# intel/rho-diffusion

Measured on AMD Instinct MI355X. Metric: denoising_steps_per_sec, higher is better.
Workload: dtype bf16; 1 GPU; DDPM reverse step, UNetv2 3D 64^3 mc=64 (BASELINE configs[2]), batch 32/GPU, bf16, LinearSchedule(1000,1e-3,0.02); global_batch=32, hip_graph=True

## Files before the change

### rho_diffusion_amd/csrc/conv.hip

```cpp
#include <cstdio>
#include <cstdlib>
#include <type_traits>

#include "conv_common.h"

#define RHO_GB_WIDE 3
#ifndef RHO_GB_BM32
#define RHO_GB_BM32 1
#endif

struct ConvK {
    const char* x1;
    const char* x2;
    const float* pre_a;
    const float* pre_b;
    const char* w;
    const float* bias;
    const char* res;
    const float* res_add;
    char* y;
    char* y2;
    int c1, c2, cin;
    int cout, coutp, split;
    int D, H, W;
// ... 984 lines not shown
                float accv = 0.0f;
                for (int q = 0; q < NTHR / PPR; ++q) accv += red[(q * PPR + piece) * (2 * PE) + e2];
                const int stat = e2 / PE, ch = co0 + piece * PE + (e2 % PE);
                q.stats[(((size_t)ns * q.tps + ts) * 2 + stat) * q.split + ch] = accv;
            }
        }
        return;
    }
#pragma unroll
    for (int jx = 0; jx < (M16 ? 4 : 2); ++jx) {
        const int pp = M16 ? tile_position16(wpos * 4 + jx, lane & 15, q.TW, q.pair_lg) : tile_position(wpos * 2 + jx, lane & 31, q.TW, q.pair_lg);
        const int pw = pp & (q.TW - 1);
        const int ph = (pp >> q.lgTW) & (q.TH - 1);
        const int pd = pp >> (q.lgTW + q.lgTH);
        const int od = od0 + pd, oh = oh0 + ph, ow = ow0 + pw;
        if (od >= q.Do || oh >= q.Ho || ow >= q.Wo) continue;
        const long long L = (((long long)n * q.Do + od) * q.Ho + oh) * q.Wo + ow;
        const long long ns = L / q.S_out;
        const long long ps = L - ns * q.S_out;
        const int j = M16 ? (jx >> 1) : jx;
#pragma unroll
        for (int mi = 0; mi < MT; ++mi) {
#pragma unroll
            for (int rx = 0; rx < (M16 ? 2 : 4); ++rx) {
                const int rg = M16 ? 2 * rx + (jx & 1) : rx;
                const int co = M16 ? co0 + wco * (BM / WCO) + 16 * (2 * mi + rx) + 4 * (lane >> 4)
                                   : co0 + wco * (BM / WCO) + mi * 32 + rg * 8 + half * 4;
                const float4 bv = *reinterpret_cast<const float4*>(q.bias + co);
                float v0 = acc[mi][j][rg * 4 + 0] + bv.x;
                float v1 = acc[mi][j][rg * 4 + 1] + bv.y;
                float v2 = acc[mi][j][rg * 4 + 2] + bv.z;
                float v3 = acc[mi][j][rg * 4 + 3] + bv.w;
                if (cl_region) {
                    if (q.res_add != nullptr) {
                        const float4 e = *reinterpret_cast<const float4*>(q.res_add + ns * q.res_add_stride + co);
                        v0 += e.x; v1 += e.y; v2 += e.z; v3 += e.w;
                    }
                    const size_t eo = (size_t)L * q.split + co;
                    if constexpr (sizeof(T) == 2) {
                        if (q.res != nullptr) {
                            const uint2 r = *reinterpret_cast<const uint2*>(q.res + eo * 2);
                            v0 += __uint_as_float(r.x << 16); v1 += __uint_as_float(r.x & 0xFFFF0000u);
                            v2 += __uint_as_float(r.y << 16); v3 += __uint_as_float(r.y & 0xFFFF0000u);
                        }
                        *reinterpret_cast<uint2*>(q.y + eo * 2) = make_uint2(pack_bf16x2(v0, v1), pack_bf16x2(v2, v3));
                    } else {
                        if (q.res != nullptr) {
                            const float4 r = *reinterpret_cast<const float4*>(q.res + eo * 4);
                            v0 += r.x; v1 += r.y; v2 += r.z; v3 += r.w;
                        }
                        *reinterpret_cast<float4*>(q.y + eo * 4) = make_float4(v0, v1, v2, v3);
                    }
                } else if (q.y2_cl) {
                    const int w2 = q.cout - q.split;
                    const size_t eo = (size_t)L * w2 + (co - q.split);
                    if (co < q.cout) {
                        if constexpr (sizeof(T) == 2) {
                            if (q.res2 != nullptr) {
                                const uint2 r = *reinterpret_cast<const uint2*>(q.res2 + eo * 2);
                                v0 += __uint_as_float(r.x << 16); v1 += __uint_as_float(r.x & 0xFFFF0000u);
                                v2 += __uint_as_float(r.y << 16); v3 += __uint_as_float(r.y & 0xFFFF0000u);
                            }
                            *reinterpret_cast<uint2*>(q.y2 + eo * 2) = make_uint2(pack_bf16x2(v0, v1), pack_bf16x2(v2, v3));
                        } else {
                            if (q.res2 != nullptr) {
                                const float4 r = *reinterpret_cast<const float4*>(q.res2 + eo * 4);
                                v0 += r.x; v1 += r.y; v2 += r.z; v3 += r.w;
                            }
                            *reinterpret_cast<float4*>(q.y2 + eo * 4) = make_float4(v0, v1, v2, v3);
                        }
                    }
                } else {
                    const float vv[4] = {v0, v1, v2, v3};
#pragma unroll
                    for (int e = 0; e < 4; ++e) {
                        if (co + e < q.cout) {
                            const size_t eo = ((size_t)ns * (q.cout - q.split) + (co + e - q.split)) * q.S_out + ps;
                            if (q.y2_f32 || sizeof(T) == 4)
                                reinterpret_cast<float*>(q.y2)[eo] = vv[e];
                            else
                                reinterpret_cast<bf16_raw*>(q.y2)[eo] = f32_to_bf16(vv[e]);
                        }
                    }
                }
            }
        }
    }
}

struct SplitMap {
    int Ho, Wo, Ho_out, Wo_out, oy_mul, oy_add, ox_mul, ox_add;
};
struct SplitOut {
    int cout, coutp, split;
    const float* bias;
    const float* res_add;
    long long res_add_stride, S_out;
    const char* res;
    char* y;
    const char* res2;
    char* y2;
};
template <typename T>
__global__ __launch_bounds__(256) void k_splitk_reduce(const float* __restrict__ slab, long long slab_stride, int ksplit, long long positions,
                                                       SplitOut o, SplitMap m) {
    const int c4 = o.coutp / 4;
    const long long item = (long long)blockIdx.x * 256 + threadIdx.x;
    if (item >= positions * c4) return;
    const long long Ls = item / c4;
    int co = (int)(item - Ls * c4) * 4;
    if (co >= o.cout) return;
    const size_t so = (size_t)Ls * o.coutp + co;
    float4 a = *reinterpret_cast<const float4*>(slab + so);
    for (int s = 1; s < ksplit; ++s) {
        const float4 b = *reinterpret_cast<const float4*>(slab + (size_t)s * slab_stride + so);
        a.x += b.x; a.y += b.y; a.z += b.z; a.w += b.w;
    }
    long long L = Ls;
    if (m.oy_mul != 1 || m.ox_mul != 1) {
        const int ow = (int)(Ls % m.Wo);
        const long long r = Ls / m.Wo;
        const int oh = (int)(r % m.Ho);
        L = ((r / m.Ho) * m.Ho_out + (oh * m.oy_mul + m.oy_add)) * m.Wo_out + (ow * m.ox_mul + m.ox_add);
    }
    const float4 bv = *reinterpret_cast<const float4*>(o.bias + co);
    float v0 = a.x + bv.x, v1 = a.y + bv.y, v2 = a.z + bv.z, v3 = a.w + bv.w;
    const bool first = co < o.split;
    if (first && o.res_add != nullptr) {
        const float4 e = *reinterpret_cast<const float4*>(o.res_add + (L / o.S_out) * o.res_add_stride + co);
        v0 += e.x; v1 += e.y; v2 += e.z; v3 += e.w;
    }
    const int width = first ? o.split : o.cout - o.split;
    const char* const res = first ? o.res : o.res2;
    char* const y = first ? o.y : o.y2;
    if (!first) co -= o.split;
    const size_t eo = (size_t)L * width + co;
    if constexpr (sizeof(T) == 2) {
        if (res != nullptr) {
            const uint2 r = *reinterpret_cast<const uint2*>(res + eo * 2);
            v0 += __uint_as_float(r.x << 16); v1 += __uint_as_float(r.x & 0xFFFF0000u);
            v2 += __uint_as_float(r.y << 16); v3 += __uint_as_float(r.y & 0xFFFF0000u);
        }
        *reinterpret_cast<uint2*>(y + eo * 2) = make_uint2(pack_bf16x2(v0, v1), pack_bf16x2(v2, v3));
    } else {
        if (res != nullptr) {
            const float4 r = *reinterpret_cast<const float4*>(res + eo * 4);
            v0 += r.x; v1 += r.y; v2 += r.z; v3 += r.w;
        }
        *reinterpret_cast<float4*>(y + eo * 4) = make_float4(v0, v1, v2, v3);
    }
}

#include "conv32.h"

namespace {

using namespace rho_conv;

struct VariantOut {
    char* buf;
    int cap;
};
thread_local VariantOut* g_variant = nullptr;

template <typename T, int KD, int KH, int KW, int BM, int MAXP, int NW, bool M16 = false, bool FSK = false, bool GNA = false>
int launch_one(const ConvK& k, dim3 grid, size_t lds, hipStream_t st) {
    if (g_variant != nullptr) {
        snprintf(g_variant->buf, (size_t)g_variant->cap, "k_conv<%s,%d,%d,%d,BM=%d,MAXP=%d,NW=%d,M16=%d>%s%s", sizeof(T) == 2 ? "bf16" : "f32",
                 KD, KH, KW, BM, MAXP, NW, (int)M16, FSK ? "+skip" : "", GNA ? "+gn_apply" : "");
        return 0;
    }
    auto fn = k_conv<T, KD, KH, KW, BM, MAXP, NW, M16, FSK, GNA>;
    if (lds > 64 * 1024) {
        hipError_t e = hipFuncSetAttribute(reinterpret_cast<const void*>(fn), hipFuncAttributeMaxDynamicSharedMemorySize, (int)lds);
        if (e != hipSuccess) return (int)e;
    }
    hipLaunchKernelGGL(fn, grid, dim3(NW * 64), lds, st, k);
    hipError_t e = hipGetLastError();
    return e == hipSuccess ? 0 : (int)e;
}

template <typename T, int KD, int KH, int KW>
int launch_bm(const ConvK& k, int BM, int np, dim3 grid, size_t lds, bool m16, hipStream_t st) {
    constexpr bool PHASE = (KH == 2 || KW == 2 || (KD == 3 && KH == 1 && KW == 1));
    if constexpr (PHASE) { if (np > 640) return RHO_E_SHAPE; }
    if constexpr (sizeof(T) == 2 && KD * KH * KW > 1 && (KD * KH * KW) % 3 == 0) {
        if (m16 && np <= 640) {
            if constexpr (KD == 3 && KH == 3 && KW == 3) {
                if (k.sk_w != nullptr) {
                    if (BM == 128) return launch_one<T, KD, KH, KW, 128, 5, 8, true, true>(k, grid, lds, st);
                    if (BM == 64) return launch_one<T, KD, KH, KW, 64, 10, 4, true, true>(k, grid, lds, st);
                }
            }
            if (BM == 128) return launch_one<T, KD, KH, KW, 128, 5, 8, true>(k, grid, lds, st);
            if (BM == 64) return launch_one<T, KD, KH, KW, 64, 10, 4, true>(k, grid, lds, st);
        }
    }
    if (k.sk_w != nullptr) return RHO_E_ARG;
    if (k.gna_g != nullptr) {
        if constexpr (KD * KH * KW == 1) {
            if (np > 640) return RHO_E_SHAPE;
            if (BM == 128) return launch_one<T, 1, 1, 1, 128, 5, 8, false, false, true>(k, grid, lds, st);
            if (BM == 64) return launch_one<T, 1, 1, 1, 64, 10, 4, false, false, true>(k, grid, lds, st);
            return launch_one<T, 1, 1, 1, 32, 10, 4, false, false, true>(k, grid, lds, st);
        }
        return RHO_E_ARG;
    }
    if (BM == 128) {
        if (np <= 640) return launch_one<T, KD, KH, KW, 128, 5, 8>(k, grid, lds, st);
        if constexpr (!PHASE) return launch_one<T, KD, KH, KW, 128, 14, 8>(k, grid, lds, st);
    }
#define RHO_CASE(bm)                                                                   \
    if (BM == bm) {                                                                    \
        if (np <= 640) return launch_one<T, KD, KH, KW, bm, 10, 4>(k, grid, lds, st);  \
        if constexpr (!PHASE) return launch_one<T, KD, KH, KW, bm, 28, 4>(k, grid, lds, st); \
    }
    RHO_CASE(32)
    RHO_CASE(64)
#undef RHO_CASE
    return RHO_E_ARG;
}

template <typename T>
int launch_taps(const rho_conv_desc& d, const ConvK& k, int BM, int np, dim3 grid, size_t lds, bool m16, hipStream_t st) {
    if (d.kd == 3 && d.kh == 3 && d.kw == 3) return launch_bm<T, 3, 3, 3>(k, BM, np, grid, lds, m16, st);
    if (d.kd == 1 && d.kh == 3 && d.kw == 3) return launch_bm<T, 1, 3, 3>(k, BM, np, grid, lds, m16, st);
    if (d.kd == 1 && d.kh == 1 && d.kw == 3) return launch_bm<T, 1, 1, 3>(k, BM, np, grid, lds, m16, st);
    if (d.kd == 1 && d.kh == 1 && d.kw == 1) return launch_bm<T, 1, 1, 1>(k, BM, np, grid, lds, m16, st);
    if (d.kd == 3 && d.kh == 2 && d.kw == 2) return launch_bm<T, 3, 2, 2>(k, BM, np, grid, lds, m16, st);
    if (d.kd == 1 && d.kh == 2 && d.kw == 2) return launch_bm<T, 1, 2, 2>(k, BM, np, grid, lds, m16, st);
    if (d.kd == 1 && d.kh == 1 && d.kw == 2) return launch_bm<T, 1, 1, 2>(k, BM, np, grid, lds, m16, st);
    if (d.kd == 3 && d.kh == 1 && d.kw == 1) return launch_bm<T, 3, 1, 1>(k, BM, np, grid, lds, m16, st);
    if (d.kd == 3 && d.kh == 1 && d.kw == 2) return launch_bm<T, 3, 1, 2>(k, BM, np, grid, lds, m16, st);
    if (d.kd == 3 && d.kh == 2 && d.kw == 1) return launch_bm<T, 3, 2, 1>(k, BM, np, grid, lds, m16, st);
    return RHO_E_ARG;
}

}

static bool m16_env_on() {
    static const bool on = !(getenv("RHO_CONV_M16") && atoi(getenv("RHO_CONV_M16")) == 0);
    return on;
}

static int conv_impl(const rho_conv_desc* dp, void* stream, int64_t* stats_tiles, int64_t* ws_want = nullptr) {
    if (!dp) return RHO_E_ARG;
    const rho_conv_desc& d = *dp;
    if (!d.x1 || !d.w || !d.bias) return RHO_E_ARG;
    if (d.dtype != RHO_F32 && d.dtype != RHO_BF16) return RHO_E_ARG;
    const int CK = d.dtype == RHO_BF16 ? 32 : 16;
    const int c2 = d.x2 ? d.c2 : 0;
    const int cin = d.c1 + c2;
    if (d.c1 <= 0 || d.c1 % CK || c2 % CK) return RHO_E_ALIGN;
    if (d.cout <= 0 || d.coutp < d.cout || d.coutp % 32 || d.split < 0 || d.split > d.cout || d.split % 32) return RHO_E_ARG;
    if (d.split > 0 && !d.y) return RHO_E_ARG;
    if (d.split < d.cout && !d.y2) return RHO_E_ARG;
    if (d.split < d.cout && d.split > 0 && d.coutp != d.cout && !d.y2_cl) return RHO_E_ARG;
    if (d.y2_cl && ((d.cout - d.split) % 4 != 0)) return RHO_E_ALIGN;
    if ((d.zs_h || d.zs_w) && (d.up_h || d.up_w || d.sh != 1 || d.sw != 1 || d.out_h <= 0 || d.out_w <= 0)) return RHO_E_ARG;
    if (d.split == d.cout && d.coutp != d.cout) return RHO_E_ARG;
    if ((d.sh != 1 && d.sh != 2) || (d.sw != 1 && d.sw != 2)) return RHO_E_ARG;
    if ((d.up_h && d.sh != 1) || (d.up_w && d.sw != 1)) return RHO_E_ARG;
    if ((d.up_h && d.kh != 3) || (d.up_w && d.kw != 3)) return RHO_E_ARG;
    if (d.n <= 0 || d.d <= 0 || d.h <= 0 || d.w_ <= 0) return RHO_E_ARG;
    if (d.ph_h < 0 || d.ph_h > 2 || d.ph_w < 0 || d.ph_w > 2) return RHO_E_ARG;
    if ((d.ph_h && ((d.kh != 2 && d.kh != 1) || d.sh != 1 || d.up_h || d.zs_h)) || (d.ph_w && ((d.kw != 2 && d.kw != 1) || d.sw != 1 || d.up_w || d.zs_w)))
        return RHO_E_ARG;
    if ((!d.ph_h && !d.phd_h && d.kh == 2) || (!d.ph_w && !d.phd_w && d.kw == 2)) return RHO_E_ARG;
    if ((d.ph_h || d.ph_w) && (d.split != d.cout || d.kd == 2)) return RHO_E_ARG;
    if (d.phd_h < 0 || d.phd_h > 2 || d.phd_w < 0 || d.phd_w > 2) return RHO_E_ARG;
    if ((d.phd_h && ((d.kh != 2 && d.kh != 1) || d.sh != 1 || d.up_h || d.zs_h || d.ph_h)) ||
        (d.phd_w && ((d.kw != 2 && d.kw != 1) || d.sw != 1 || d.up_w || d.zs_w || d.ph_w)))
        return RHO_E_ARG;
    if ((d.ph_h || d.phd_h || d.ph_w || d.phd_w) && d.kd * d.kh * d.kw == 1) return RHO_E_ARG;
    if ((d.phd_h || d.phd_w) && (d.kd == 2 || d.pre_a)) return RHO_E_ARG;

    if (conv32_applies(d)) {
        if (stats_tiles) { *stats_tiles = conv32_wps(d); return 0; }
        if (ws_want) { *ws_want = 0; return 0; }
        if (g_variant != nullptr) { snprintf(g_variant->buf, (size_t)g_variant->cap, "k_conv32<bf16>"); return 0; }
        if (d.stats && d.split != d.cout) return RHO_E_ARG;
        return launch_conv32(d, as_stream(stream));
    }

    const int hv = d.zs_h ? d.out_h : d.h, wv = d.zs_w ? d.out_w : d.w_;
    const int ho = (d.ph_h || d.phd_h) ? d.h : d.up_h ? d.h * 2 : (hv + 2 * (d.kh / 2) - d.kh) / d.sh + 1;
    const int wo = (d.ph_w || d.phd_w) ? d.w_ : d.up_w ? d.w_ * 2 : (wv + 2 * (d.kw / 2) - d.kw) / d.sw + 1;
    const int ho_out = d.ph_h ? 2 * ho : ho, wo_out = d.ph_w ? 2 * wo : wo;
    const int n_phase = (d.ph_h ? 2 : 1) * (d.ph_w ? 2 : 1);
    const int phase_idx = (d.ph_h ? d.ph_h - 1 : 0) * (d.ph_w ? 2 : 1) + (d.ph_w ? d.ph_w - 1 : 0);
    const int dout = d.d;

    ConvK k{};
    int gridz = d.n;
    k.pad_h = d.kh == 1 ? 0 : d.ph_h ? 2 - d.ph_h : d.phd_h ? d.phd_h - 1 : d.kh / 2;
    k.pad_w = d.kw == 1 ? 0 : d.ph_w ? 2 - d.ph_w : d.phd_w ? d.phd_w - 1 : d.kw / 2;
    k.iy_mul = d.phd_h ? 2 : 1; k.iy_add = d.phd_h ? d.phd_h - 1 : 0;
    k.ix_mul = d.phd_w ? 2 : 1; k.ix_add = d.phd_w ? d.phd_w - 1 : 0;
    k.oy_mul = d.ph_h ? 2 : 1; k.oy_add = d.ph_h ? d.ph_h - 1 : 0;
    k.ox_mul = d.ph_w ? 2 : 1; k.ox_add = d.ph_w ? d.ph_w - 1 : 0;
    if (d.kd == 1 && d.kh == 1 && d.kw == 1) {
        if (d.sh != 1 || d.sw != 1 || d.up_h || d.up_w) return RHO_E_ARG;
        k.D = 1; k.H = 1; k.W = d.n * d.d * d.h * d.w_;
        k.Do = 1; k.Ho = 1; k.Wo = k.W;
        gridz = 1;
    } else if (d.kd == 1) {
        k.D = d.n * d.d; k.H = hv; k.W = wv;
        k.Do = k.D; k.Ho = ho; k.Wo = wo;
        gridz = 1;
    } else {
        k.D = d.d; k.H = hv; k.W = wv;
        k.Do = dout; k.Ho = ho; k.Wo = wo;
    }
    k.Hs = k.H; k.Ws = k.W;
    if (d.zs_h) k.Hs = d.h;
    if (d.zs_w) k.Ws = d.w_;
    if (d.phd_h) k.Hs = 2 * d.h;
    if (d.phd_w) k.Ws = 2 * d.w_;
    k.zs_h = d.zs_h; k.zs_w = d.zs_w;
    k.y2_cl = d.y2_cl; k.res2 = (const char*)d.res2;
    if ((long long)d.n * d.d * d.h * d.w_ * (d.phd_h ? 2 : 1) * (d.phd_w ? 2 : 1) >= (1LL << 31) || (long long)d.n * dout * ho_out * wo_out >= (1LL << 31)) return RHO_E_SHAPE;
    k.S_in = (long long)d.d * d.h * d.w_ * (d.phd_h ? 2 : 1) * (d.phd_w ? 2 : 1);
    k.S_out = (long long)dout * ho_out * wo_out;
    k.Ho_out = (d.kd == 1 && d.kh == 1 && d.kw == 1) ? 1 : ho_out;
    k.Wo_out = (d.kd == 1 && d.kh == 1 && d.kw == 1) ? k.Wo : wo_out;

    int BM = 32;
    if (d.coutp % 128 == 0 && (d.split % 128 == 0)) BM = 128;
    else if (d.coutp % 64 == 0 && (d.split % 64 == 0)) BM = 64;

    const size_t lds_cap = 160 * 1024;
    const int taps = d.kd * d.kh * d.kw;
    {
        static const int bm64_chunks = getenv("RHO_BM64_MAX_CHUNKS") ? atoi(getenv("RHO_BM64_MAX_CHUNKS")) : 0;
        if (BM == 128 && bm64_chunks > 0 && d.kd == 3 && taps > 1 && cin / CK <= bm64_chunks) BM = 64;
    }
    const bool m16 = d.dtype == RHO_BF16 && taps > 1 && taps % 3 == 0 && d.sh == 1 && d.sw == 1 && !d.up_h && !d.up_w;
    const int WSLOTS = (taps % 3 == 0) ? ((((BM == 128 && m16) || (RHO_GB_BM32 && BM == 32)) && RHO_GB_WIDE == 3 && taps % 9 == 0) ? 9 : 3) : 2;
    int np_cap = (int)((lds_cap - (size_t)WSLOTS * BM * PITCH) / PITCH);
    if (np_cap > 28 * 64) np_cap = 28 * 64;
    TileChoice t = choose_tile(d, k.D, k.Do, k.Ho, k.Wo, 640);
    if (!t.ok) t = choose_tile(d, k.D, k.Do, k.Ho, k.Wo, np_cap);
    if (!t.ok) return RHO_E_SHAPE;

    k.x1 = (const char*)d.x1; k.x2 = (const char*)d.x2; k.pre_a = d.pre_a; k.pre_b = d.pre_b;
    k.w = (const char*)d.w; k.bias = d.bias; k.res = (const char*)d.res; k.res_add = d.res_add;
    k.y = (char*)d.y; k.y2 = (char*)d.y2;
    k.c1 = d.c1; k.c2 = c2; k.cin = cin;
    k.cout = d.cout; k.coutp = d.coutp; k.split = d.split;
    k.res_add_stride = d.res_add_stride > 0 ? d.res_add_stride : d.split;
    k.sh = d.sh; k.sw = d.sw; k.up_h = d.up_h; k.up_w = d.up_w; k.pre_silu = d.pre_silu; k.y2_f32 = d.y2_f32;
    k.TD = t.TD; k.TH = t.TH; k.TW = t.TW; k.ID = t.ID; k.IH = t.IH; k.IW = t.IW; k.NP = t.NP;
    k.tiles_h = cdiv(k.Ho, t.TH); k.tiles_w = cdiv(k.Wo, t.TW);
    k.lgTW = 0; k.lgTH = 0;
    while ((1 << k.lgTW) < t.TW) ++k.lgTW;
    while ((1 << k.lgTH) < t.TH) ++k.lgTH;
    if ((1 << k.lgTW) != t.TW || (1 << k.lgTH) != t.TH) return RHO_E_SHAPE;
    k.inv_ihw = 1.0f / (float)(t.IH * t.IW); k.inv_iw = 1.0f / (float)t.IW;
    k.pair_lg = -1;
    if (t.TW == 8 && d.sw == 1 && d.sh == 1 && !d.up_h && !d.up_w) {
        int lgTH = 0;
        while ((1 << lgTH) < t.TH) ++lgTH;
        for (int b = 0; b < 5 && k.pair_lg < 0; ++b) {
            const long long delta = (b < lgTH) ? (long long)(1 << b) * t.IW : (long long)(1 << (b - lgTH)) * t.IH * t.IW;
            if ((1 << b) < t.TD * t.TH && delta % 16 == 8) k.pair_lg = b;
        }
    }
    if (d.pre_a && !d.pre_b) return RHO_E_ARG;

    const long long tiles = (long long)cdiv(k.Do, t.TD) * k.tiles_h * k.tiles_w;
    if (tiles > 0x7FFFFFFFLL || d.coutp / BM > 65535 || gridz > 65535) return RHO_E_SHAPE;
    k.cofast = (d.coutp / BM > 1 && tiles % 8 == 0) ? 1 : 0;
    dim3 grid((unsigned)tiles, (unsigned)(d.coutp / BM), (unsigned)gridz);
    int64_t tps_geo = 0;
    if (d.kd == 3) tps_geo = tiles * n_phase;
    else if (taps == 1 && k.S_out % 256 == 0 && t.TW == 256) tps_geo = k.S_out / 256;
    const int64_t tps = (d.split == d.cout && d.split > 0) ? tps_geo : 0;
    if (stats_tiles) { *stats_tiles = tps; return 0; }
    int ksplit = 1;
    const long long positions = (long long)k.Do * k.Ho * k.Wo;
    {
        const long long wgs = tiles * (d.coutp / BM);
        const int chunks = cin / CK;
        static const bool split_env = !(getenv("RHO_CONV_SPLITK") && atoi(getenv("RHO_CONV_SPLITK")) == 0);
        if (split_env && d.kd == 1 && (d.split == d.cout || d.y2_cl) && !d.stats && !d.gna_g && wgs <= 128 && chunks >= 4) {
            int want = (int)(512 / wgs);
            if (want > 16) want = 16;
            const int per = taps == 1 ? 4 : 2;
            if (want > chunks / per) want = chunks / per;
            if (ws_want) { *ws_want = want >= 2 ? (int64_t)want * positions * d.coutp * (int64_t)sizeof(float) : 0; return 0; }
            if (d.ws != nullptr && want >= 2) {
                const long long fit = d.ws_bytes / (positions * d.coutp * (long long)sizeof(float));
                if (fit < want) want = (int)fit;
                if (want >= 2) ksplit = want;
            }
        } else if (ws_want) { *ws_want = 0; return 0; }
    }
    k.ksplit = ksplit; k.slab = (float*)d.ws; k.slab_stride = positions * d.coutp;
    if (ksplit > 1) grid.z = (unsigned)ksplit;
    k.stats = nullptr; k.tps = 1;
    if (d.stats) {
        if (tps <= 0) return RHO_E_ARG;
        k.stats = d.stats; k.tps = (int)tps;
        k.stats_off = phase_idx * (int)tiles;
    }
    k.gnb_x1 = nullptr;
    k.gna_g = nullptr;
    if (d.gna_g) {
        const int pe = d.dtype == RHO_BF16 ? 8 : 4;
        if (taps != 1 || d.res || d.res2 || d.stats || !d.gnb_x1 || !d.gnb_a || !d.gnb_b || !d.gna_cA || !d.gna_cP || !d.gna_cQ || d.split <= 0 || d.cout % 32 ||
            d.gnb_c1 <= 0 || d.gnb_c1 > d.cout || d.gnb_c1 % 32 || ((d.gnb_c1 < d.cout) != (d.gnb_x2 != nullptr)) || tps_geo <= 0 ||
            (d.split < d.cout && (!d.y2_cl || (d.cout - d.split) % pe != 0)) || d.gnb_silu < 0 || d.gnb_silu > 1 || n_phase != 1)
            return RHO_E_ARG;
        k.gnb_x1 = (const char*)d.gnb_x1; k.gnb_x2 = (const char*)d.gnb_x2; k.gnb_a = d.gnb_a; k.gnb_b = d.gnb_b;
        k.gnb_c1 = d.gnb_c1; k.gnb_silu = d.gnb_silu;
        k.gna_g = (const char*)d.gna_g; k.gna_cA = d.gna_cA; k.gna_cP = d.gna_cP; k.gna_cQ = d.gna_cQ;
        k.tps = (int)tps_geo;
    } else if (d.gnb_x1) {
        if (!d.stats || !d.gnb_a || !d.gnb_b || d.gnb_c1 <= 0 || d.gnb_c1 > d.split || d.gnb_c1 % 32 || (d.split - d.gnb_c1) % 32 ||
            ((d.gnb_c1 < d.split) != (d.gnb_x2 != nullptr)))
            return RHO_E_ARG;
        k.gnb_x1 = (const char*)d.gnb_x1; k.gnb_x2 = (const char*)d.gnb_x2; k.gnb_a = d.gnb_a; k.gnb_b = d.gnb_b;
        k.gnb_c1 = d.gnb_c1; k.gnb_silu = d.gnb_silu;
    }
    size_t lds = (size_t)t.NP * PITCH + (size_t)WSLOTS * BM * PITCH;
    k.sk_w = nullptr;
    size_t lds_sk = 0;
    if (d.sk_w) {
        if (!d.sk_x1 || d.sk_c1 <= 0 || d.sk_c1 % CK || d.sk_c2 < 0 || d.sk_c2 % CK || ((d.sk_c2 > 0) != (d.sk_x2 != nullptr))) return RHO_E_ARG;
        if (!(m16 && m16_env_on() && d.kd == 3 && d.kh == 3 && d.kw == 3 && t.NP <= 640 && (BM == 64 || BM == 128) && d.split == d.cout &&
              !d.zs_h && !d.zs_w && !d.ph_h && !d.ph_w && !d.phd_h && !d.phd_w))
            return RHO_E_ARG;
        k.sk_x1 = (const char*)d.sk_x1; k.sk_x2 = (const char*)d.sk_x2; k.sk_w = (const char*)d.sk_w; k.sk_bias = d.sk_bias;
        k.sk_c1 = d.sk_c1; k.sk_c2 = d.sk_c2;
        lds_sk = (size_t)2 * 256 * PITCH + (size_t)2 * BM * PITCH;
    }
    k.coef_off = 0;
// ... 49 lines not shown
```

### rho_diffusion_amd/engine/unet_engine.py

```python
from __future__ import annotations

import os
from collections import namedtuple
from typing import Callable, Dict, List, Optional, Tuple

import torch
from torch import nn

from .. import hip
from ..hip import check, ptr
from . import ops
from .backward_plan import BackwardBuilder
from .forward_plan import ForwardBuilder
from .weights import _ConvW, _HeadDgradW

Tensor = torch.Tensor


PlanSwitches = namedtuple("PlanSwitches", "materialize_act materialize_min_cout phase_upsample phase_upsample_bwd phase_min_wgs fold_skip "
                                     "s2_split s2_split_bwd fuse_gn_bwd gemm_ends direct_ends fuse_skip_dgrad")


class UNetEngine:
    def __init__(self, model: nn.Module, dtype: torch.dtype):
        self.model = model
        self.dtype = dtype
        p = next(model.parameters())
        hip.require_gpu(p, "UNet parameters")
        hip.load()
        self.device = p.device
        self.dims = model.dims
        self.mc = model.model_channels
        self.ssn = bool(model.use_scale_shift_norm)
        self.act = int(getattr(model, "act_code", 1))
        self._plans: Dict[tuple, "_Plan"] = {}
        self._convs: List[_ConvW] = []
        self._aux_weights: list = []
        self._conv_of: Dict[int, _ConvW] = {}
        self._film_blocks: List[nn.Module] = []
        self._omega: Optional[Tensor] = None
        self._cond_dev = None
        self._param_version = -1
        self._ptr_sig = None
        self._prep_table = None
        self._prep_sig = None
        self._prep_eager: List[_ConvW] = []
        self._last_train_plan: Optional["_Plan"] = None
        with torch.inference_mode(False):
            self._collect()
            self.refresh_weights(force=True)

    def _conv(self, mod: nn.Module, row_src: Optional[Tensor] = None) -> _ConvW:
        key = id(mod)
        if key not in self._conv_of:
            cw = _ConvW(mod.weight, mod.bias, self.dtype, row_src)
            self._conv_of[key] = cw
            self._convs.append(cw)
        return self._conv_of[key]

    def _conv_as_gemm(self, mod: nn.Module, cls) -> _ConvW:
        key = (id(mod), cls.__name__)
        if key not in self._conv_of:
            cw = cls(mod.weight, mod.bias, self.dtype)
            self._conv_of[key] = cw
            self._convs.append(cw)
        return self._conv_of[key]

    def _head_dgrad(self, mod: nn.Module) -> "_HeadDgradW":
        key = (id(mod), "_HeadDgradW")
        if key not in self._conv_of:
            hw = _HeadDgradW(mod.weight, self.dtype)
            self._conv_of[key] = hw
            self._aux_weights.append(hw)
        return self._conv_of[key]

    def _qkv_row_src(self, blk) -> Tensor:
        c, h = blk.channels, blk.num_heads
        ch = c // h
        idx = torch.arange(3 * c, dtype=torch.int64)
        if not blk.use_new_attention_order:
            part = idx // c
            head = (idx % c) // ch
            i = idx % ch
            idx = head * 3 * ch + part * ch + i
        return idx.to(torch.int32).to(self.device)

    def _collect(self) -> None:
        from ..models.unet_v2 import AttentionBlock, Downsample, ResBlock, Upsample
        m = self.model
        for mod in m.modules():
            if isinstance(mod, ResBlock):
                self._film_blocks.append(mod)
                self._conv(mod.in_layers[2])
                self._conv(mod.out_layers[3])
                if not isinstance(mod.skip_connection, nn.Identity):
                    self._conv(mod.skip_connection)
            elif isinstance(mod, AttentionBlock):
                self._conv(mod.qkv, self._qkv_row_src(mod))
                self._conv(mod.proj_out)
            elif isinstance(mod, Downsample):
                if mod.use_conv:
                    self._conv(mod.op)
            elif isinstance(mod, Upsample):
                if mod.use_conv:
                    self._conv(mod.conv)
        self._conv(m.input_blocks[0][0])
        self._conv(m.out[2])
        self._film_off: Dict[int, int] = {}
        off = 0
        for blk in self._film_blocks:
            self._film_off[id(blk)] = off
            off += blk.emb_layers[1].weight.shape[0]
        self.film_total = off
        e = 4 * self.mc
        self.film_w = torch.empty(off, e, dtype=torch.float32, device=self.device)
        self.film_b = torch.empty(off, dtype=torch.float32, device=self.device)

    def _versions(self) -> int:
        return sum(p._version for p in self.model.parameters())

    def _pointer_signature(self) -> int:
        return hash(tuple(p.data_ptr() for p in self.model.parameters()))

    def refresh_weights(self, force: bool = False) -> None:
        sig = self._pointer_signature()
        if self._ptr_sig is not None and sig != self._ptr_sig:
            self._plans.clear()
            self._last_train_plan = None
            force = True
        self._ptr_sig = sig
        v = self._versions()
        if not force and v == self._param_version:
            return
        allw = self._convs + self._aux_weights
        lsig = tuple(cw.layout_signature() for cw in allw) + tuple(blk.emb_layers[1].weight.data_ptr() for blk in self._film_blocks)
        if self._prep_table is None or self._prep_sig != lsig:
            table = ops.PrepTable(self.device)
            self._prep_eager = [cw for cw in allw if not cw.prep_into(table)]
            off = 0
            for blk in self._film_blocks:
                lin = blk.emb_layers[1]
                n = lin.weight.shape[0]
                table.add_vec(lin.weight.detach().reshape(-1), self.film_w[off:off + n].reshape(-1))
                table.add_vec(lin.bias.detach(), self.film_b[off:off + n])
                off += n
            self._prep_table, self._prep_sig = table, lsig
        self._prep_table.launch()
        for cw in self._prep_eager:
            cw.refresh()
        self._param_version = v

    def omega(self) -> Tensor:
        if self._omega is None:
            self._omega = ops.sinusoid_frequencies(self.mc, 10000, self.device)
        return self._omega

    def err_flag(self) -> Tensor:
        if getattr(self, "_err_flag", None) is None:
            self._err_flag = torch.zeros(1, dtype=torch.int32, device=self.device)
        return self._err_flag

    def check_errors(self) -> None:
        if getattr(self, "_err_flag", None) is not None:
            v = int(self._err_flag.item())
            if v & 2:
                self._err_flag.zero_()
                raise IndexError("MultiEmbeddings: a label value is not in the parameter space (conditioning.py:132)")

    def cond_device_tables(self):
        from ..models.conditioning import MultiEmbeddings
        fn = getattr(self.model, "cond_fn", None)
        if not isinstance(fn, MultiEmbeddings) or fn.parameter_space is None or len(fn.embedding_layers) == 0:
            return None
        weights = [layer.weight for layer in fn.embedding_layers.values()]
        sig = tuple(w.data_ptr() for w in weights)
        if self._cond_dev is not None and self._cond_dev["sig"] == sig:
            return self._cond_dev
        keys = list(fn.embedding_layers.keys())
        if len(keys) > 16:
            return None
        vals, off = [], [0]
        for k in keys:
            v = torch.tensor(fn.parameter_space[k]).to(torch.float32)
            vals.append(v)
            off.append(off[-1] + v.numel())
        dev = self.device
        self._cond_dev = dict(sig=sig, nkeys=len(keys), weights=weights,
                              space=torch.cat(vals).to(dev).contiguous(),
                              key_off=torch.tensor(off, dtype=torch.int32, device=dev),
                              tables=torch.tensor(list(sig), dtype=torch.int64, device=dev))
        return self._cond_dev

    def param_order(self) -> List[nn.Parameter]:
        emb = list(self.model.time_embed.parameters())
        for blk in self._film_blocks:
            emb.extend(blk.emb_layers[1].parameters())
        if getattr(self.model, "cond_fn", None) is not None:
            emb.extend(self.model.cond_fn.parameters())
        emb_ids = {id(p_) for p_ in emb}
        main = [p_ for p_ in self.model.parameters() if id(p_) not in emb_ids]
        return emb + main

    def forward(self, x: Tensor, timesteps: Tensor, y: Optional[Tensor] = None,
                t_scalar_dev: Optional[Tensor] = None, train: bool = False) -> Tensor:
        hip.require_gpu(x, "x")
        if x.dtype != torch.float32:
            x = x.float()
        x = x.contiguous()
        self.refresh_weights()
        key = (tuple(x.shape), y is not None, bool(train)) + self._plan_signature()
        plan = self._plans.get(key)
        if plan is None:
            with torch.inference_mode(False), torch.no_grad():
                plan = self._plans[key] = _Plan(self, tuple(x.shape), y is not None, bool(train))
        if train:
            self._last_train_plan = plan
        return plan.run(x, timesteps, y, t_scalar_dev)

    _PLAN_ENV = ("RHO_TRAIN_MATERIALIZE", "RHO_MATERIALIZE_MIN_COUT", "RHO_PHASE_UPSAMPLE", "RHO_PHASE_UPSAMPLE_BWD", "RHO_PHASE_MIN_WGS",
                 "RHO_FOLD_SKIP", "RHO_S2_SPLIT", "RHO_S2_SPLIT_BWD", "RHO_FUSE_GN_BWD", "RHO_GEMM_ENDS", "RHO_DIRECT_ENDS",
                 "RHO_FUSE_SKIP_DGRAD")

    @staticmethod
    def _plan_switches() -> PlanSwitches:
        return PlanSwitches(
            materialize_act=os.environ.get("RHO_TRAIN_MATERIALIZE", "1") != "0",
            materialize_min_cout=int(os.environ.get("RHO_MATERIALIZE_MIN_COUT", "256")),
            phase_upsample=os.environ.get("RHO_PHASE_UPSAMPLE", "1") != "0",
            phase_upsample_bwd=os.environ.get("RHO_PHASE_UPSAMPLE_BWD", "1") != "0",
            phase_min_wgs=int(os.environ.get("RHO_PHASE_MIN_WGS", "256")),
            fold_skip=os.environ.get("RHO_FOLD_SKIP", "1") != "0",
            s2_split=os.environ.get("RHO_S2_SPLIT", "1") != "0",
            s2_split_bwd=os.environ.get("RHO_S2_SPLIT_BWD", "1") != "0",
            fuse_gn_bwd=int(os.environ.get("RHO_FUSE_GN_BWD", "128")),
            gemm_ends=os.environ.get("RHO_GEMM_ENDS", "1") != "0",
            direct_ends=os.environ.get("RHO_DIRECT_ENDS", "1") != "0",
            fuse_skip_dgrad=os.environ.get("RHO_FUSE_SKIP_DGRAD", "1") != "0")

    def _plan_signature(self) -> tuple:
        ck = tuple(bool(b.use_checkpoint) for b in self._film_blocks)
        env = tuple(os.environ.get(k) for k in self._PLAN_ENV)
        drop = bool(self.model.training) if any(float(getattr(b, "dropout", 0.0) or 0.0) > 0.0 for b in self._film_blocks) else None
        return (ck, ops.deterministic(), env, drop)

    def drop_plans(self, train_only: bool = False) -> None:
        self._plans = {k: v for k, v in self._plans.items() if train_only and not k[2]}
        self._last_train_plan = None

    def backward(self, dpred: Tensor, on_ready: Optional[Callable[[List[nn.Parameter]], None]] = None) -> None:
        plan = self._last_train_plan
        if plan is None:
            raise hip.RhoHipError("backward() without a preceding forward(train=True)")
        with torch.no_grad():
            plan.run_backward(dpred, on_ready)


class _Plan:

    def __init__(self, eng: UNetEngine, xshape: Tuple[int, ...], has_y: bool, train: bool):
        self.eng, self.train, self.has_y = eng, train, has_y
        self.sw = eng._plan_switches()
        self.L = hip.lib()
        self.B, self.xshape = xshape[0], xshape
        self.ops: List[Callable[[int], int]] = []
        self.info: List[dict] = []
        self.keep: List[object] = []
        self.tstats: Dict[int, Tuple[Tensor, int]] = {}
        self.nodes: List[dict] = []
        self.fwd_descs: List[object] = []
        self.wgrad_descs: List[tuple] = []
        self.cond_src = None
        self.drop_active = bool(eng.model.training) and any(float(getattr(b, "dropout", 0.0) or 0.0) > 0.0 for b in eng._film_blocks)
        self.drop_ctr = torch.zeros(1, dtype=torch.int64, device=eng.device) if self.drop_active else None
        self.drop_delta = 0
        self.drop_nodes: List[dict] = []
        self.bwd: List[Callable[[int], int]] = []
        self.bwd_info: List[dict] = []
        self.bwd_marks: List[Tuple[int, List[nn.Parameter]]] = []
        ForwardBuilder(self).build()
        if train:
            BackwardBuilder(self).build()
        ws = ops.attach_conv_workspace(self.fwd_descs, eng.device)
        if ws is not None:
            self.keep.append(ws)

    def nbytes(self) -> int:
        seen, tot = set(), 0
        for t in self.keep:
            if torch.is_tensor(t) and t.data_ptr() not in seen:
                seen.add(t.data_ptr())
                tot += t.numel() * t.element_size()
        return tot + int(getattr(self, "pool_bytes", 0))

    def variants(self) -> List[str]:
        out = [ops.conv_variant(d) for d in self.fwd_descs]
        out += [ops.conv_wgrad_variant(d, w_) for d, w_ in self.wgrad_descs]
        return out

    def run(self, x: Tensor, timesteps: Optional[Tensor], y: Optional[Tensor], t_scalar_dev: Optional[Tensor]) -> Tensor:
        eng = self.eng
        m = eng.model
        if x.data_ptr() != self.x_in.data_ptr():
            self.x_in.copy_(x)
        te0, te2 = m.time_embed[0], m.time_embed[2]
        self.cond_src = None
        self.cond_dev = None
        if self.cond is not None:
            if y.dim() == 2 and tuple(y.shape) == tuple(self.emb.shape):
                self.cond.copy_(y.to(self.cond.device))
            else:
                if y.dim() == 1:
                    assert y.shape == (x.shape[0],)
                else:
                    assert y.shape[0] == self.emb.shape[0]
                cd = eng.cond_device_tables()
                if cd is not None:
                    yf = y.to(device=self.cond.device, dtype=torch.float32).contiguous()
                    if yf.dim() == 2 and yf.shape[1] != cd["nkeys"]:
                        raise hip.RhoHipError(f"labels have {yf.shape[1]} columns, the parameter space has {cd['nkeys']} keys")
                    self.keep_y = yf
                    check(self.L.rho_multi_embed(ptr(yf), 1 if yf.dim() == 1 else yf.shape[1], ptr(cd["space"]), ptr(cd["key_off"]),
                                                 ptr(cd["tables"]), cd["nkeys"], self.B, self.cond.shape[1], ptr(self.cond),
                                                 ptr(self.cond_idx), ptr(eng.err_flag()), hip.stream()), "rho_multi_embed")
                    self.cond_dev = cd
                else:
                    with (torch.enable_grad() if self.train else torch.no_grad()):
                        c = m.cond_fn(y)
                    self.cond_src = c if (self.train and c.requires_grad) else None
                    self.cond.copy_(c.detach())
        if t_scalar_dev is not None:
            tptr, tsptr = None, ptr(t_scalar_dev)
        else:
            hip.require_gpu(timesteps, "timesteps")
            self.t_in.copy_(timesteps.reshape(-1))
            tptr, tsptr = ptr(self.t_in), None
        check(self.L.rho_timestep_embed(ptr(eng.omega()), tptr, tsptr, ptr(te0.weight), ptr(te0.bias), ptr(te2.weight), ptr(te2.bias),
                                        ptr(self.cond), ptr(self.sin_in), ptr(self.emb_h), ptr(self.emb), self.B, eng.mc,
                                        self.emb.shape[1], eng.act, hip.stream()), "rho_timestep_embed")
        s = hip.stream()
        if self.drop_active:
            check(self.L.rho_step_advance(None, ptr(self.drop_ctr), self.drop_delta, s), "rho_step_advance")
        for op in self.ops:
            rc = op(s)
            if rc != 0:
                check(rc, "UNet plan launch")
        return self.out

    def run_backward(self, dpred: Tensor, on_ready=None) -> None:
        eng = self.eng
        for p_ in eng.model.parameters():
            if p_.grad is None:
                p_.grad = torch.zeros_like(p_)
        self.dpred_in.copy_(dpred.reshape(self.dpred_in.shape))
        s = hip.stream()
        marks: Dict[int, list] = {}
        for i, ps in self.bwd_marks:
            marks.setdefault(i, []).extend(ps)
        for i, op in enumerate(self.bwd):
            rc = op(s)
            if rc != 0:
                check(rc, "UNet backward plan launch")
            if on_ready is not None and (i + 1) in marks:
                on_ready(marks[i + 1])
        if self.cond_dev is not None:
            cd = self.cond_dev
            gsig = tuple(w.grad.data_ptr() for w in cd["weights"])
            if getattr(self, "_gp_sig", None) != gsig:
                self._gp = torch.tensor(list(gsig), dtype=torch.int64, device=self.demb.device)
                self._gp_sig = gsig
            gp = self._gp
            check(self.L.rho_multi_embed_bwd(ptr(self.demb), ptr(self.cond_idx), ptr(gp), cd["nkeys"], self.B, self.demb.shape[1], s),
                  "rho_multi_embed_bwd")
        elif self.cond_src is not None:
            with torch.enable_grad():
                self.cond_src.backward(self.demb)
        if on_ready is not None:
            on_ready([])

    def profile(self, repeats: int = 3, backward: bool = False) -> List[dict]:
        s = hip.stream()
        lst, infos = (self.bwd, self.bwd_info) if backward else (self.ops, self.info)
        tot = [0.0] * len(lst)
        for _ in range(repeats):
            evs = [(torch.cuda.Event(enable_timing=True), torch.cuda.Event(enable_timing=True)) for _ in lst]
            for op, (e0, e1) in zip(lst, evs):
                e0.record()
                rc = op(s)
                e1.record()
                if rc != 0:
                    check(rc, "UNet plan launch (profile)")
# ... 5 lines not shown
```

Before: 8.663 steps/s.

## Add dedicated MFMA GEMM kernel for 1x1x1 bf16 convolutions

```diff
diff --git a/rho_diffusion_amd/csrc/conv.hip b/rho_diffusion_amd/csrc/conv.hip
--- a/rho_diffusion_amd/csrc/conv.hip
+++ b/rho_diffusion_amd/csrc/conv.hip
@@ -1160,6 +1160,7 @@
 }
 
 #include "conv32.h"
+#include "gemm1x1.h"
 
 namespace {
 
@@ -1291,6 +1292,13 @@
         return launch_conv32(d, as_stream(stream));
     }
 
+    if (gemm1x1_applies(d)) {
+        if (stats_tiles) { *stats_tiles = gemm1x1_stats_tiles(d); return 0; }
+        if (ws_want) { *ws_want = 0; return 0; }
+        if (g_variant != nullptr) { snprintf(g_variant->buf, (size_t)g_variant->cap, "k_gemm1x1<bf16,256x%d>", G1_BN); return 0; }
+        return launch_gemm1x1(d, as_stream(stream));
+    }
+
     const int hv = d.zs_h ? d.out_h : d.h, wv = d.zs_w ? d.out_w : d.w_;
     const int ho = (d.ph_h || d.phd_h) ? d.h : d.up_h ? d.h * 2 : (hv + 2 * (d.kh / 2) - d.kh) / d.sh + 1;
     const int wo = (d.ph_w || d.phd_w) ? d.w_ : d.up_w ? d.w_ * 2 : (wv + 2 * (d.kw / 2) - d.kw) / d.sw + 1;
diff --git a/rho_diffusion_amd/csrc/gemm1x1.h b/rho_diffusion_amd/csrc/gemm1x1.h
--- /dev/null
+++ b/rho_diffusion_amd/csrc/gemm1x1.h
@@ -0,0 +1,269 @@
+#pragma once
+#include <cstdlib>
+#include <type_traits>
+
+#include "conv_common.h"
+
+#define G1_BN 128
+#define G1_ROWS (256 + G1_BN)
+#define G1_BUF (G1_ROWS * 128)
+#define G1_NBUF 3
+#define G1_DMA (G1_ROWS / 64)
+
+struct Gemm1K {
+    const char* x;
+    const char* w;
+    const float* bias;
+    const char* res;
+    char* y;
+    char* y2;
+    float* stats;
+    int cin, cout, split;
+    int ctiles;
+    int tps;
+    long long S;
+};
+
+__device__ __forceinline__ void g1_unpack8(const uint4& r, float* v) {
+    v[0] = __uint_as_float(r.x << 16); v[1] = __uint_as_float(r.x & 0xFFFF0000u);
+    v[2] = __uint_as_float(r.y << 16); v[3] = __uint_as_float(r.y & 0xFFFF0000u);
+    v[4] = __uint_as_float(r.z << 16); v[5] = __uint_as_float(r.z & 0xFFFF0000u);
+    v[6] = __uint_as_float(r.w << 16); v[7] = __uint_as_float(r.w & 0xFFFF0000u);
+}
+
+__global__ __launch_bounds__(512) void k_gemm1x1(const Gemm1K p) {
+    extern __shared__ __attribute__((aligned(16))) char smem[];
+    const int tid = threadIdx.x;
+    const int lane = tid & 63;
+    const int wave = tid >> 6;
+    const int wp = wave & 3;
+    const int wc = wave >> 2;
+    const int fi = lane & 15;
+    const int fg = lane >> 4;
+
+    int wg;
+    {
+        const int nwg = (int)gridDim.x, L = (int)blockIdx.x;
+        const int xcd = L & 7, q = nwg >> 3, r = nwg & 7;
+        wg = (xcd < r ? xcd * (q + 1) : r * (q + 1) + (xcd - r) * q) + (L >> 3);
+    }
+    const int ct = wg % p.ctiles, bt = wg / p.ctiles;
+    const int co0 = ct * G1_BN;
+    const long long pos0 = (long long)bt * 256;
+
+    const char* src[G1_DMA];
+#pragma unroll
+    for (int j = 0; j < G1_DMA; ++j) {
+        const int R = j * 64 + wave * 8 + (lane >> 3);
+        const int lp = (lane & 7) ^ ((R >> 1) & 7);
+        const int r = R & 15, f = (R >> 4) & 3, w64 = (R >> 6) & 3;
+        const int m = w64 * 64 + (r >> 2) * 16 + f * 4 + (r & 3);
+        if (j < 4) src[j] = p.x + (size_t)(pos0 + m) * (size_t)p.cin * 2 + lp * 16;
+        else src[j] = p.w + (size_t)(co0 + (m & (G1_BN - 1))) * (size_t)p.cin * 2 + lp * 16;
+    }
+    const unsigned ldsw = __builtin_amdgcn_readfirstlane((unsigned)(size_t)(__attribute__((address_space(3))) char*)smem + (unsigned)wave * 1024u);
+    auto glds16 = [&](const char* gsrc, unsigned lds_dst) {
+        asm volatile("s_mov_b32 m0, %1\n\ts_nop 0\n\tglobal_load_lds_dwordx4 %0, off" : : "v"(gsrc), "s"(lds_dst) : "memory");
+    };
+    auto issue = [&](int buf) {
+#pragma unroll
+        for (int j = 0; j < G1_DMA; ++j) {
+            glds16(src[j], ldsw + (unsigned)buf * G1_BUF + (unsigned)j * 8192u);
+            src[j] += 128;
+        }
+    };
+
+    const int offk0 = ((fg) ^ (fi >> 1)) * 16, offk1 = ((4 + fg) ^ (fi >> 1)) * 16;
+    const int offp = (wp * 64 + fi) * 128;
+    const int offc = (256 + wc * 64 + fi) * 128;
+
+    f32x4_t acc[4][4];
+#pragma unroll
+    for (int a = 0; a < 4; ++a)
+#pragma unroll
+        for (int b = 0; b < 4; ++b) acc[a][b] = f32x4_t{0.0f, 0.0f, 0.0f, 0.0f};
+
+    const int nk = p.cin >> 6;
+    const bool yreg = co0 < p.split;
+    auto kloop = [&](auto YREG) {
+        constexpr bool W_IS_A = decltype(YREG)::value;
+        issue(0);
+        if (nk > 1) issue(1);
+        int cur = 0, nxt = 2;
+        for (int k = 0; k < nk; ++k) {
+            if (k + 1 < nk) asm volatile("s_waitcnt vmcnt(%0)" : : "n"(G1_DMA) : "memory");
+            else asm volatile("s_waitcnt vmcnt(0)" ::: "memory");
+            __syncthreads();
+            if (k + 2 < nk) issue(nxt);
+            const char* const base = smem + cur * G1_BUF;
+#pragma unroll
+            for (int kk = 0; kk < 2; ++kk) {
+                const int ok = kk ? offk1 : offk0;
+                bf16x8_t fp[4], fc[4];
+#pragma unroll
+                for (int f = 0; f < 4; ++f) {
+                    fp[f] = __builtin_bit_cast(bf16x8_t, *reinterpret_cast<const uint4*>(base + offp + f * 2048 + ok));
+                    fc[f] = __builtin_bit_cast(bf16x8_t, *reinterpret_cast<const uint4*>(base + offc + f * 2048 + ok));
+                }
+#pragma unroll
+                for (int a = 0; a < 4; ++a)
+#pragma unroll
+                    for (int b = 0; b < 4; ++b) {
+                        if constexpr (W_IS_A) acc[a][b] = __builtin_amdgcn_mfma_f32_16x16x32_bf16(fc[a], fp[b], acc[a][b], 0, 0, 0);
+                        else acc[a][b] = __builtin_amdgcn_mfma_f32_16x16x32_bf16(fp[b], fc[a], acc[a][b], 0, 0, 0);
+                    }
+            }
+            cur = cur == G1_NBUF - 1 ? 0 : cur + 1;
+            nxt = nxt == G1_NBUF - 1 ? 0 : nxt + 1;
+        }
+    };
+    if (yreg) kloop(std::true_type{});
+    else kloop(std::false_type{});
+
+    if (yreg) {
+        const int cl = co0 + wc * 64 + fg * 16;
+        float bia[16];
+#pragma unroll
+        for (int a = 0; a < 4; ++a) {
+            const float4 b4 = *reinterpret_cast<const float4*>(p.bias + cl + a * 4);
+            bia[a * 4 + 0] = b4.x; bia[a * 4 + 1] = b4.y; bia[a * 4 + 2] = b4.z; bia[a * 4 + 3] = b4.w;
+        }
+        size_t eo[4];
+        uint4 rr[4][2];
+#pragma unroll
+        for (int b = 0; b < 4; ++b) {
+            const long long P = pos0 + wp * 64 + (fi >> 2) * 16 + b * 4 + (fi & 3);
+            eo[b] = ((size_t)P * (size_t)p.split + (size_t)cl) * 2;
+            rr[b][0] = rr[b][1] = make_uint4(0u, 0u, 0u, 0u);
+            if (p.res != nullptr) {
+                rr[b][0] = *reinterpret_cast<const uint4*>(p.res + eo[b]);
+                rr[b][1] = *reinterpret_cast<const uint4*>(p.res + eo[b] + 16);
+            }
+        }
+        float ssum[16], ssq[16];
+#pragma unroll
+        for (int e = 0; e < 16; ++e) ssum[e] = ssq[e] = 0.0f;
+#pragma unroll
+        for (int b = 0; b < 4; ++b) {
+            float v[16];
+#pragma unroll
+            for (int a = 0; a < 4; ++a)
+#pragma unroll
+                for (int j = 0; j < 4; ++j) v[a * 4 + j] = acc[a][b][j] + bia[a * 4 + j];
+            if (p.res != nullptr) {
+                float rv[16];
+                g1_unpack8(rr[b][0], rv);
+                g1_unpack8(rr[b][1], rv + 8);
+#pragma unroll
+                for (int e = 0; e < 16; ++e) v[e] += rv[e];
+            }
+            typedef unsigned int u32x4_nt __attribute__((ext_vector_type(4)));
+            const u32x4_nt o0 = {pack_bf16x2(v[0], v[1]), pack_bf16x2(v[2], v[3]), pack_bf16x2(v[4], v[5]), pack_bf16x2(v[6], v[7])};
+            const u32x4_nt o1 = {pack_bf16x2(v[8], v[9]), pack_bf16x2(v[10], v[11]), pack_bf16x2(v[12], v[13]), pack_bf16x2(v[14], v[15])};
+            __builtin_nontemporal_store(o0, reinterpret_cast<u32x4_nt*>(p.y + eo[b]));
+            __builtin_nontemporal_store(o1, reinterpret_cast<u32x4_nt*>(p.y + eo[b] + 16));
+            if (p.stats != nullptr) {
+                float sv[16];
+                g1_unpack8(make_uint4(o0.x, o0.y, o0.z, o0.w), sv);
+                g1_unpack8(make_uint4(o1.x, o1.y, o1.z, o1.w), sv + 8);
+#pragma unroll
+                for (int e = 0; e < 16; ++e) {
+                    ssum[e] += sv[e];
+                    ssq[e] = fmaf(sv[e], sv[e], ssq[e]);
+                }
+            }
+        }
+        if (p.stats != nullptr) {
+#pragma unroll
+            for (int e = 0; e < 16; ++e) {
+#pragma unroll
+                for (int o = 1; o < 16; o <<= 1) {
+                    ssum[e] += __shfl_xor(ssum[e], o, 64);
+                    ssq[e] += __shfl_xor(ssq[e], o, 64);
+                }
+            }
+            __syncthreads();
+            float* const red = reinterpret_cast<float*>(smem);
+            if (fi == 0) {
+#pragma unroll
+                for (int e = 0; e < 16; ++e) {
+                    red[(wp * 2 + 0) * G1_BN + wc * 64 + fg * 16 + e] = ssum[e];
+                    red[(wp * 2 + 1) * G1_BN + wc * 64 + fg * 16 + e] = ssq[e];
+                }
+            }
+            __syncthreads();
+            if (tid < 2 * G1_BN) {
+                const int stat = tid / G1_BN, ch = tid % G1_BN;
+                float a = 0.0f;
+#pragma unroll
+                for (int q = 0; q < 4; ++q) a += red[(q * 2 + stat) * G1_BN + ch];
+                p.stats[((size_t)bt * 2 + stat) * (size_t)p.split + co0 + ch] = a;
+            }
+        }
+        return;
+    }
+    const int ns = bt / p.tps;
+    const long long ps = (long long)(bt % p.tps) * 256 + wp * 64 + fg * 16;
+    const int w2 = p.cout - p.split;
+    float bia[4];
+#pragma unroll
+    for (int a = 0; a < 4; ++a) bia[a] = p.bias[co0 + wc * 64 + (fi >> 2) * 16 + a * 4 + (fi & 3)];
+#pragma unroll
+    for (int a = 0; a < 4; ++a) {
+        const int co = co0 + wc * 64 + (fi >> 2) * 16 + a * 4 + (fi & 3);
+        const float bv = bia[a];
+        char* const dst = p.y2 + (((size_t)ns * (size_t)w2 + (size_t)(co - p.split)) * (size_t)p.S + (size_t)ps) * 2;
+        float v[16];
+#pragma unroll
+        for (int b = 0; b < 4; ++b)
+#pragma unroll
+            for (int j = 0; j < 4; ++j) v[b * 4 + j] = acc[a][b][j] + bv;
+        *reinterpret_cast<uint4*>(dst) = make_uint4(pack_bf16x2(v[0], v[1]), pack_bf16x2(v[2], v[3]), pack_bf16x2(v[4], v[5]), pack_bf16x2(v[6], v[7]));
+        *reinterpret_cast<uint4*>(dst + 16) =
+            make_uint4(pack_bf16x2(v[8], v[9]), pack_bf16x2(v[10], v[11]), pack_bf16x2(v[12], v[13]), pack_bf16x2(v[14], v[15]));
+    }
+}
+
+static bool gemm1x1_on() {
+    const char* e = getenv("RHO_GEMM1X1");
+    return !(e && atoi(e) == 0);
+}
+
+static bool gemm1x1_applies(const rho_conv_desc& d) {
+    if (!gemm1x1_on()) return false;
+    if (d.dtype != RHO_BF16 || d.kd != 1 || d.kh != 1 || d.kw != 1 || d.sh != 1 || d.sw != 1 || d.up_h || d.up_w) return false;
+    if (d.x2 || d.pre_a || d.pre_b || d.res_add || d.y2_f32 || d.y2_cl || d.res2 || d.gnb_x1 || d.gna_g || d.sk_w) return false;
+    if (d.zs_h || d.zs_w || d.ph_h || d.ph_w || d.phd_h || d.phd_w) return false;
+    if (d.c1 % 64 || d.coutp != d.cout || d.cout % G1_BN || d.split % G1_BN) return false;
+    if ((d.split > 0 && !d.y) || (d.split < d.cout && !d.y2) || (d.stats && d.split != d.cout)) return false;
+    const uintptr_t al = (uintptr_t)d.x1 | (uintptr_t)d.w | (uintptr_t)d.bias | (uintptr_t)d.y | (uintptr_t)d.y2 | (uintptr_t)d.res;
+    if (al & 15) return false;
+    const long long S = (long long)d.d * d.h * d.w_, total = S * d.n;
+    if (total % 256 || total >= (1LL << 31)) return false;
+    if ((d.stats || d.split < d.cout) && S % 256) return false;
+    const long long wgs = total / 256 * (d.cout / G1_BN);
+    if (wgs > 0x7FFFFFFFLL) return false;
+    if (d.split == d.cout && !d.stats && wgs <= 128 && d.c1 / 32 >= 4) return false;
+    return true;
+}
+static int64_t gemm1x1_stats_tiles(const rho_conv_desc& d) {
+    const long long S = (long long)d.d * d.h * d.w_;
+    return (d.split == d.cout && S % 256 == 0) ? S / 256 : 0;
+}
+static int launch_gemm1x1(const rho_conv_desc& d, hipStream_t st) {
+    Gemm1K k{};
+    k.x = (const char*)d.x1; k.w = (const char*)d.w; k.bias = d.bias; k.res = (const char*)d.res;
+    k.y = (char*)d.y; k.y2 = (char*)d.y2; k.stats = d.stats;
+    k.cin = d.c1; k.cout = d.cout; k.split = d.split;
+    k.ctiles = d.cout / G1_BN;
+    k.S = (long long)d.d * d.h * d.w_;
+    k.tps = (k.S % 256 == 0) ? (int)(k.S / 256) : 1;
+    const long long wgs = k.S * d.n / 256 * k.ctiles;
+    const size_t lds = (size_t)G1_NBUF * G1_BUF;
+    static const hipError_t attr = hipFuncSetAttribute(reinterpret_cast<const void*>(k_gemm1x1), hipFuncAttributeMaxDynamicSharedMemorySize, (int)lds);
+    if (attr != hipSuccess) return (int)attr;
+    hipError_t e;
+    hipLaunchKernelGGL(k_gemm1x1, dim3((unsigned)wgs), dim3(512), lds, st, k);
+    e = hipGetLastError();
+    return e == hipSuccess ? 0 : (int)e;
+}
diff --git a/rho_diffusion_amd/engine/unet_engine.py b/rho_diffusion_amd/engine/unet_engine.py
--- a/rho_diffusion_amd/engine/unet_engine.py
+++ b/rho_diffusion_amd/engine/unet_engine.py
@@ -18,7 +18,7 @@
 
 
 PlanSwitches = namedtuple("PlanSwitches", "materialize_act materialize_min_cout phase_upsample phase_upsample_bwd phase_min_wgs fold_skip "
-                                     "s2_split s2_split_bwd fuse_gn_bwd gemm_ends direct_ends fuse_skip_dgrad")
+                                     "s2_split s2_split_bwd fuse_gn_bwd gemm_ends direct_ends fuse_skip_dgrad gemm1x1")
 
 
 class UNetEngine:
@@ -219,7 +219,7 @@
 
     _PLAN_ENV = ("RHO_TRAIN_MATERIALIZE", "RHO_MATERIALIZE_MIN_COUT", "RHO_PHASE_UPSAMPLE", "RHO_PHASE_UPSAMPLE_BWD", "RHO_PHASE_MIN_WGS",
                  "RHO_FOLD_SKIP", "RHO_S2_SPLIT", "RHO_S2_SPLIT_BWD", "RHO_FUSE_GN_BWD", "RHO_GEMM_ENDS", "RHO_DIRECT_ENDS",
-                 "RHO_FUSE_SKIP_DGRAD")
+                 "RHO_FUSE_SKIP_DGRAD", "RHO_GEMM1X1")
 
     @staticmethod
     def _plan_switches() -> PlanSwitches:
@@ -235,7 +235,8 @@
             fuse_gn_bwd=int(os.environ.get("RHO_FUSE_GN_BWD", "128")),
             gemm_ends=os.environ.get("RHO_GEMM_ENDS", "1") != "0",
             direct_ends=os.environ.get("RHO_DIRECT_ENDS", "1") != "0",
-            fuse_skip_dgrad=os.environ.get("RHO_FUSE_SKIP_DGRAD", "1") != "0")
+            fuse_skip_dgrad=os.environ.get("RHO_FUSE_SKIP_DGRAD", "1") != "0",
+            gemm1x1=os.environ.get("RHO_GEMM1X1", "1") != "0")
 
     def _plan_signature(self) -> tuple:
         ck = tuple(bool(b.use_checkpoint) for b in self._film_blocks)
```

Measured after the change: 8.779 steps/s (median of 6 runs). 1.3% higher.
